# zhouxuguang/GNXRayTracer

Measured on AMD Instinct MI355X. Metric: Mrays/sec + wall-clock to 1024spp, dragon Cornell 1920×1080, higher is better.
Workload: dtype f32; 1 GPU; cfg3: Cornell + synthetic 100000-tri mesh (stand-in for absent dragon.3d), Glass+Metal, PathIntegrator maxDepth 8 rr 1 spatial, Halton(1024), 1920x1080; passes_in_flight=4, sub_passes=56, spp_rendered=1024, gather=n/a, world_size=1, backend=none, devices_visible=1

## Files before the change

gnxraytracer_amd/csrc/api.hip:

```cpp
#include <hip/hip_runtime.h>

#include <chrono>
#include <cstdio>
#include <cstdlib>
#include <memory>
#include <mutex>
#include <string>
#include <thread>
#include <vector>

#include "host_scene.h"
#include "kernels.hip.h"
#include "trace4_kernel.hip.h"
#include "hlbvh_build.hip.h"
#include "refit_kernel.hip.h"
#include "material_kernel.hip.h"
#include "rebuild_kernel.hip.h"
#include "env_build_kernel.hip.h"
#include "media_kernel.hip.h"
#include "texture_build_kernel.hip.h"
#include "li_kernel.hip.h"
#include "views_kernel.hip.h"
#include "shade_query_kernel.hip.h"
#include "aov_kernel.hip.h"
#include "kernel_instances.h"

using namespace gnxr;

#define X(M, L, S, T) extern template GX_WHITTED_SIGNATURE(M, L, S, T)
GX_WHITTED_INSTANCES(X)
#undef X
#define X(M, L, ST, T) extern template GX_VOL_SIGNATURE(M, L, ST, T)
GX_VOL_INSTANCES(X)
#undef X
#define X(M, L) extern template GX_SHADE_KIND_SIGNATURE(M, L)
GX_SHADE_KIND_INSTANCES(X)
#undef X
extern template GX_BSDF_QUERY_SIGNATURE(LM_ALL)
extern template GX_LIGHT_SAMPLE_QUERY_SIGNATURE(LT_ALL)
extern template GX_LIGHT_LE_QUERY_SIGNATURE(LT_ALL)
extern template GX_TRACE_CLOSEST_CODE_SIGNATURE(32)
extern template GX_TRACE_CLOSEST_CODE_SIGNATURE(64)
#define X(M) extern template GX_AOV_RESOLVE_SIGNATURE(M)
GX_AOV_INSTANCES(X)
#undef X

#include "api_common.hip.h"
#include "api_scene.hip.h"
#include "api_hlbvh.hip.h"
#include "api_probes.hip.h"
#include "api_device_call.hip.h"
#include "api_render.hip.h"

extern "C" {

int gnxr_init(int device_id) {
    int n = 0;
    hipError_t e = hipGetDeviceCount(&n);
    if (e != hipSuccess || n <= 0) { set_error("no HIP device available; libgnxr has no CPU fallback"); return GNXR_ERR_NO_DEVICE; }
// ... 394 lines not shown
```

gnxraytracer_amd/csrc/api_common.hip.h:

```cpp
#pragma once

namespace { int hip_status(hipError_t e); }
#define HIP_TRY(expr)                                                                                   \
    do {                                                                                                \
        hipError_t e_ = (expr);                                                                         \
        if (e_ != hipSuccess) {                                                                         \
            set_error("%s failed: %s (%s:%d)", #expr, hipGetErrorString(e_), __FILE__, __LINE__);       \
            return hip_status(e_);                                                                      \
        }                                                                                               \
    } while (0)

namespace {

int hip_status(hipError_t e) {
    if (e == hipErrorOutOfMemory) return GNXR_ERR_OOM;
    if (e == hipErrorNoDevice || e == hipErrorInvalidDevice || e == hipErrorInsufficientDriver || e == hipErrorNotInitialized) return GNXR_ERR_NO_DEVICE;
    return GNXR_ERR_RUNTIME;
}

int g_device = -1;
std::vector<int> g_devices;
std::vector<char> g_peer_ok;
int g_num_cus = 256;
int g_profiling = 0;
// ... 24 lines not shown
struct Knobs {
    static int env_int(const char *name, int unset) { const char *e = getenv(name); return e ? atoi(e) : unset; }
    static bool env_set(const char *name) { return getenv(name) != nullptr; }
#define GX_ONCE(type, expr) do { static const type v = (expr); return v; } while (0)
    static int trace_blocks_per_cu() { const int v = env_int("GNXR_TRACE_BLOCKS_PER_CU", 0); return v >= 1 && v <= 8 ? v : 0; }
    static int grid_blocks_per_cu() { const int v = env_int("GNXR_GRID_BLOCKS_PER_CU", 0); return v >= 1 && v <= 4096 ? v : 0; }
    static int trace_lds_levels() { GX_ONCE(int, env_set("GNXR_TRACE_LDS_LEVELS") ? std::max(2, env_int("GNXR_TRACE_LDS_LEVELS", 0)) : 64); }
    static int trace_chunk() { GX_ONCE(int, env_set("GNXR_TRACE_CHUNK") ? std::max(64, env_int("GNXR_TRACE_CHUNK", 0) / 64 * 64) : kTraceChunk); }
    static bool leaf_box_table() { GX_ONCE(bool, env_set("GNXR_LEAF_BOX_TABLE")); }
    static int regions() { GX_ONCE(int, env_int("GNXR_REGIONS", 0)); }
    static bool pipeline() { GX_ONCE(bool, env_int("GNXR_PIPELINE", 1) != 0); }
    static int pipe_cut() { GX_ONCE(int, env_int("GNXR_PIPE_CUT", -1)); }
    static int loop_lag() { GX_ONCE(int, env_int("GNXR_LOOP_LAG", -1)); }
    static int shade_blocks_per_cu() { GX_ONCE(int, env_set("GNXR_SHADE_BLOCKS_PER_CU") ? std::max(1, env_int("GNXR_SHADE_BLOCKS_PER_CU", 0)) : 32); }
    static int shade_lds_dims() { GX_ONCE(int, env_set("GNXR_SHADE_LDS_DIMS") ? std::max(0, std::min(128, env_int("GNXR_SHADE_LDS_DIMS", 0))) : 64); }
    static bool shade_lds_tables() { GX_ONCE(bool, env_int("GNXR_SHADE_LDS_TABLES", 1) != 0); }
    static int shade_streams() { GX_ONCE(int, env_int("GNXR_SHADE_STREAMS", -1)); }
    static bool vol_pack() { GX_ONCE(bool, env_int("GNXR_VOL_PACK", 1) != 0); }
#undef GX_ONCE
    static int volmedia_step_cap() { return env_set("GNXR_VOLMEDIA_STEP_CAP") ? std::max(0, env_int("GNXR_VOLMEDIA_STEP_CAP", 0)) : 64; }
    static bool no_escape_queue() { return env_set("GNXR_NO_ESCAPE_QUEUE"); }
    static bool no_material_queues() { return env_set("GNXR_NO_MATERIAL_QUEUES"); }
    static bool no_narrow_shade() { return env_set("GNXR_NO_NARROW_SHADE"); }
    static bool host_light_grid() { return env_set("GNXR_HOST_LIGHT_GRID"); }
    static bool binary_bvh() { return env_set("GNXR_BINARY_BVH"); }
};

int ensure_device() {
    if (g_device >= 0) { HIP_TRY(hipSetDevice(g_device)); return GNXR_OK; }
    int n = 0;
    hipError_t e = hipGetDeviceCount(&n);
    if (e != hipSuccess || n <= 0) {
        set_error("no HIP device available (%s); libgnxr has no CPU fallback", e != hipSuccess ? hipGetErrorString(e) : "0 devices");
        return GNXR_ERR_NO_DEVICE;
    }
    int dev = 0;
    HIP_TRY(hipGetDevice(&dev));
    hipDeviceProp_t prop;
    HIP_TRY(hipGetDeviceProperties(&prop, dev));
    g_num_cus = prop.multiProcessorCount > 0 ? prop.multiProcessorCount : 256;
    g_device = dev;
    if (const int v = Knobs::trace_blocks_per_cu()) g_trace_blocks_per_cu = v;
    if (const int v = Knobs::grid_blocks_per_cu()) g_grid_bpc = v;
    return GNXR_OK;
}

// ... 32 lines not shown
```

gnxraytracer_amd/csrc/api_render.hip.h:

```cpp
#pragma once

struct TraceLaunch {
    int entries;
    int lds_entries;
    bool spill_needed;
    size_t lds;
    int n_top;
    int blocks;
};
static TraceLaunch trace_launch(const gnxr_scene *s, bool wide, bool spheres, long long total) {
    TraceLaunch t;
    t.entries = wide ? s->cs.stack4_need + 1 : s->cs.bvh_max_depth + 2;
    const int per_cu = g_trace_blocks_per_cu;
    const size_t fixed_b = wide ? (size_t)(kRayRecDwords + (spheres ? 1 : 0)) * kRqStride * sizeof(int) + (size_t)kTopCache * 128 + kOrderTableBytes : 0;
    t.lds_entries = std::min(std::min(t.entries, Knobs::trace_lds_levels()), std::max(2, (int)(((160 * 1024) / per_cu - 1024 - fixed_b) / (kBlock * sizeof(int)))));
    t.spill_needed = t.entries > t.lds_entries;
    t.lds = (size_t)t.lds_entries * kBlock * sizeof(int) + fixed_b;
    t.n_top = (int)std::min<size_t>(kTopCache, s->cs.root4 >= 0 ? s->cs.nodes4.size() : 0);
    t.blocks = (int)std::min<long long>((long long)g_num_cus * per_cu, (total + kBlock - 1) / kBlock);
    return t;
}

static int count_local_rows(const gnxr_render_params *p) {
    int rows = 0;
// ... 257 lines not shown
        record_ptrs(vol_alt_rec, ps.rec);
        ps.state = vol_alt_state.p; ps.orig = vol_alt_orig.p;
    }
    return ps;
}

struct RenderRun {
    gnxr_scene *s;
    RenderState &st;
    hipStream_t stream;
    const RenderPlan &pl;
    const RaySource *src;
    const ViewSource *views;
    DScene sc;
    DRender r;
    PathArrays pa;
    VolArrays va;
    WhittedArrays wa;
    DMediaTables mt;
    Counters *dctr;
    KernelTimer timer;
    const bool timing = (g_profiling & 1) != 0, count_wide = (g_profiling & 4) != 0, counting = (g_profiling & 2) != 0 && !count_wide;
    bool spheres;
    bool list_media = false;
    int n_lights, n_scene_media;
    unsigned long long rays_closest = 0, rays_any = 0, rays_mis = 0, media_segments = 0;
    unsigned long long new_paths = 0;
    unsigned int launches = 0, passes = 0, loop_iterations = 0;

    RenderRun(gnxr_scene *scene, hipStream_t stream_, const RenderPlan &plan, const RaySource *src_, const ViewSource *views_, const DScene &sc_, const DRender &r_)
        : s(scene), st(scene->st), stream(stream_), pl(plan), src(src_), views(views_), sc(sc_), r(r_), pa(st.path_arrays()), va(st.vol_arrays()),
          wa(st.whitted_arrays(plan, (int)scene->cs.desc_lights.size())), mt(scene->media_tables()), dctr(scene->counters.p), spheres(scene->cs.n_spheres > 0),
          n_lights((int)scene->cs.desc_lights.size()), n_scene_media((int)scene->cs.media.size()) {}

    void launch_trace(TraceWork w, int n_sh, int n_mis, bool count_rays = true);
    void compact(int mode, const int *qin, int nin, const unsigned char *keys, int nout, int nscatter, unsigned int *totals, int *o0, int *o1, int *o2, int *o3 = nullptr, int split = 0,
                 const unsigned *n_dev = nullptr, unsigned kind_queue = 0x01010101u);
    int shade_stage(const int *q_in, int n, int *q_out, const unsigned *n_dev);
    void raygen(const PathArrays &at, long long u0, int kk, unsigned char *medium_keys);
    void resolve(const PathArrays &at, long long u0, int kk);
    void bind_set(const VolPackSet &ps);
};

void RenderRun::launch_trace(TraceWork w, int n_sh, int n_mis, bool count_rays) {
    long long total = (long long)w.n_closest + w.n_nee;
    if (total <= 0) return;
// ... 34 lines not shown
        (void)hipMemsetAsync(st.tile_desc.p, 0, st.tile_desc.n * sizeof(unsigned long long), stream);
        st.compact_seq = 0;
    }
    const unsigned seq = ++st.compact_seq;
    const CompactScratch cs{st.tile_desc.p, tiles, st.compact_ticket.p + (seq & 1u), st.compact_ticket.p + ((seq + 1u) & 1u), seq};
    const bool hitclass = mode == COMPACT_HITCLASS;
    const int *hit = hitclass ? (const int *)st.hit.p : nullptr;
    const unsigned char *cls = hitclass ? (const unsigned char *)s->tri_class.p : nullptr;
#define GX_COMPACT(M, N, NS) hipLaunchKernelGGL((k_compact<M, N, NS>), dim3(g), dim3(kCompactBlock), 0, stream, qin, nin, keys, cs, totals, o0, o1, o2, o3, hit, cls, kind_queue, split, n_dev, dctr)
    if (mode == COMPACT_FLAGS) {
        if (nout == 5) { if (nscatter == 3) GX_COMPACT(COMPACT_FLAGS, 5, 3); else GX_COMPACT(COMPACT_FLAGS, 5, 2); }
        else { if (nscatter == 3) GX_COMPACT(COMPACT_FLAGS, 4, 3); else GX_COMPACT(COMPACT_FLAGS, 4, 2); }
    } else if (hitclass) { if (nout == 4) GX_COMPACT(COMPACT_HITCLASS, 4, 4); else GX_COMPACT(COMPACT_HITCLASS, 3, 3); }
    else if (nout == 4) GX_COMPACT(COMPACT_CLASS, 4, 4);
    else GX_COMPACT(COMPACT_CLASS, 3, 3);
#undef GX_COMPACT
    launches += 1;
}
static int compact_stalled(const Counters &c) {
    if (!c.compact_stall) return GNXR_OK;
    set_error("queue compaction: a tile waited for its predecessors beyond the poll limit (k_compact); the render was abandoned");
    return GNXR_ERR_RUNTIME;
}

int RenderRun::shade_stage(const int *q_in, int n, int *q_out, const unsigned *n_dev) {
    if (timing) timer.begin(2, stream);
    const int *qk = pl.queue_kernel;
    const int n_classes = qk[3] != SHADE_Q_NONE ? 4 : 3;
    compact(COMPACT_HITCLASS, q_in, n, st.pclass.p, n_classes, n_classes, &dctr->q_class[0], st.queue_c0.p, st.queue_c1.p, st.queue_c2.p, st.queue_c3.p, 0, n_dev, pl.kind_queue);
    int *qc[4] = {st.queue_c0.p, st.queue_c1.p, st.queue_c2.p, st.queue_c3.p};
    dim3 g(grid_for(n, Knobs::shade_blocks_per_cu())), b(kBlock);
    const int sdims = std::min<int>(Knobs::shade_lds_dims(), (int)s->cs.prime_sums.size() - 1);
    const int snperm = sdims > 0 ? s->cs.prime_sums[sdims] : 0;
    const bool shade_lds_tabs = Knobs::shade_lds_tables();
    const int lmats = (shade_lds_tabs && s->cs.materials.size() <= 12) ? (int)s->cs.materials.size() : 0;
    const int llights = (shade_lds_tabs && n_lights > 0 && n_lights <= 16) ? n_lights : 0;
    const size_t slds = (sdims > 0 ? ((((size_t)snperm * 2 + 15) & ~(size_t)15) + (size_t)sdims * 32) : 0) + (size_t)lmats * sizeof(DMaterial) + (size_t)llights * sizeof(DLight);
    const int shade_streams = Knobs::shade_streams();
    int n_class_kernels = 0;
    for (int q = 0; q < 4; ++q) n_class_kernels += qk[q] != SHADE_Q_NONE ? 1 : 0;
    const bool fork = (shade_streams < 0 ? n_class_kernels >= 3 : (shade_streams != 0 && n_class_kernels >= 2)) && s->aux_stream[0] && s->aux_stream[1];
    hipStream_t cst[4] = {stream, stream, stream, stream};
    if (fork) {
        HIP_TRY(hipEventRecord(s->ev_fork, stream));
        HIP_TRY(hipStreamWaitEvent(s->aux_stream[0], s->ev_fork, 0));
        HIP_TRY(hipStreamWaitEvent(s->aux_stream[1], s->ev_fork, 0));
        cst[1] = s->aux_stream[0]; cst[2] = s->aux_stream[1]; cst[3] = s->aux_stream[1];
    }
    const bool area_only = pl.area_only, area_env_only = pl.area_env_only;
#define GX_SHADE_K(K, C) hipLaunchKernelGGL(K, g, b, slds, cst[C], sc, r, pa, (const int *)qc[C], (const unsigned int *)&dctr->q_class[C], sdims, snperm, lmats, llights)
#define GX_SHADE(LMV, LTV, C) do { if (spheres) GX_SHADE_K((k_shade<LMV, LTV, true>), C); else GX_SHADE_K((k_shade<LMV, LTV, false>), C); } while (0)
#define GX_SHADE_TEX(LTV) do { if (spheres) GX_SHADE_K((k_shade<LM_ALL, LTV, true, true>), 3); else GX_SHADE_K((k_shade<LM_ALL, LTV, false, true>), 3); } while (0)
    const int light_set = area_only ? 0 : ((area_env_only && !spheres && !(pl.class_mask & 8)) ? 1 : 2);
#define GX_SHADE_LM(LMV, C) do { \
        if (light_set == 0) GX_SHADE(LMV, LT_AREA, C); \
        else if (light_set == 1) GX_SHADE_K((k_shade<LMV, LT_AREA | LT_ENV, false>), C); \
        else GX_SHADE(LMV, LT_ALL, C); } while (0)
#define GX_SHADE_NARROW(LMV, C) do { \
        if (light_set == 0) GX_SHADE_K((k_shade<LMV, LT_AREA, false>), C); \
        else if (light_set == 1) GX_SHADE_K((k_shade<LMV, LT_AREA | LT_ENV, false>), C); \
        else GX_SHADE_K((k_shade<LMV, LT_ALL, false>), C); } while (0)
    for (int q = 0; q < 4; ++q) {
        switch (qk[q]) {
        case SHADE_Q_DIFFUSE: GX_SHADE_LM(LM_DIFFUSE, q); break;
        case SHADE_Q_GLOSSY: GX_SHADE_LM(LM_GLOSSY, q); break;
        case SHADE_Q_CONDUCTOR: GX_SHADE_NARROW(LM_CONDUCTOR, q); break;
        case SHADE_Q_ROUGH_DIELECTRIC: GX_SHADE_NARROW(LM_ROUGH_DIELECTRIC, q); break;
        case SHADE_Q_ALL: GX_SHADE_LM(LM_ALL, q); break;
        case SHADE_Q_TEX: if (light_set == 0) GX_SHADE_TEX(LT_AREA); else GX_SHADE_TEX(LT_ALL); break;
        case SHADE_Q_ESCAPE:
            if (area_env_only) hipLaunchKernelGGL((k_shade_escape<LT_AREA | LT_ENV>), g, b, 0, cst[q], sc, pa, (const int *)qc[q], (const unsigned int *)&dctr->q_class[q]);
            else hipLaunchKernelGGL((k_shade_escape<LT_ALL>), g, b, 0, cst[q], sc, pa, (const int *)qc[q], (const unsigned int *)&dctr->q_class[q]);
            break;
        default: continue;
        }
        ++launches;
    }
#undef GX_SHADE_NARROW
#undef GX_SHADE_LM
#undef GX_SHADE_TEX
#undef GX_SHADE
#undef GX_SHADE_K
    if (fork) {
        HIP_TRY(hipEventRecord(s->ev_join[0], s->aux_stream[0]));
        HIP_TRY(hipEventRecord(s->ev_join[1], s->aux_stream[1]));
        HIP_TRY(hipStreamWaitEvent(stream, s->ev_join[0], 0));
        HIP_TRY(hipStreamWaitEvent(stream, s->ev_join[1], 0));
    }
    compact(COMPACT_FLAGS, q_in, n, st.pflags.p, 4, 2, &dctr->q_next, q_out, st.queue_nee.p, nullptr, nullptr, 0, n_dev);
    if (timing) timer.end(stream);
    return GNXR_OK;
}

void RenderRun::raygen(const PathArrays &at, long long u0, int kk, unsigned char *medium_keys) {
    const int n_new = (int)(pl.unit * kk);
    if (views) hipLaunchKernelGGL(k_raygen_views, dim3(grid_for(n_new)), dim3(kBlock), 0, stream, sc, r, (const DCamera *)st.view_cams.p, at, n_new, (int)u0, medium_keys);
    else if (!src) hipLaunchKernelGGL(k_raygen, dim3(grid_for(n_new)), dim3(kBlock), 0, stream, sc, r, at, n_new, (int)u0);
    else hipLaunchKernelGGL(k_raygen_rays, dim3(grid_for(n_new)), dim3(kBlock), 0, stream, sc, r, at, reinterpret_cast<const float4 *>(src->rays + u0),
                            reinterpret_cast<const int4 *>(src->samples + u0), n_new, n_scene_media, medium_keys, dctr, u0);
}
void RenderRun::resolve(const PathArrays &at, long long u0, int kk) {
    if (!src) hipLaunchKernelGGL(k_resolve, dim3(grid_for(r.npix)), dim3(kBlock), 0, stream, at, st.accum.p, r.npix, kk);
    else hipLaunchKernelGGL(k_store_li, dim3(grid_for(kk)), dim3(kBlock), 0, stream, (const float4 *)at.L, reinterpret_cast<const int4 *>(src->samples + u0), r,
                            n_scene_media, kk, reinterpret_cast<float4 *>(src->L) + u0);
}
// ... 474 lines not shown
```

gnxraytracer_amd/csrc/device_bsdf.h:

```cpp
#pragma once
#include "device_sampler.h"

namespace gnxr {

GX_DEV float cos_theta(V3 w) { return w.z; }
GX_DEV float cos2_theta(V3 w) { return w.z * w.z; }
GX_DEV float abs_cos_theta(V3 w) { return fabsf(w.z); }
GX_DEV float sin2_theta(V3 w) { return fmaxf(0.f, 1.f - cos2_theta(w)); }
GX_DEV float sin_theta(V3 w) { return gx_sqrt(sin2_theta(w)); }
GX_DEV float tan_theta(V3 w) { return sin_theta(w) / cos_theta(w); }
GX_DEV float tan2_theta(V3 w) { return sin2_theta(w) / cos2_theta(w); }
GX_DEV float cos_phi(V3 w) { float s = sin_theta(w); return (s == 0) ? 1 : clampf(w.x / s, -1, 1); }
GX_DEV float sin_phi(V3 w) { float s = sin_theta(w); return (s == 0) ? 0 : clampf(w.y / s, -1, 1); }
GX_DEV float cos2_phi(V3 w) { return cos_phi(w) * cos_phi(w); }
GX_DEV float sin2_phi(V3 w) { return sin_phi(w) * sin_phi(w); }
GX_DEV bool same_hemisphere(V3 w, V3 wp) { return w.z * wp.z > 0; }
GX_DEV V3 reflect(V3 wo, V3 n) { return -wo + 2 * dot(wo, n) * n; }
GX_DEV bool refract(V3 wi, V3 n, float eta, V3 *wt) {
    float cosThetaI = dot(n, wi);
    float sin2ThetaI = fmaxf(0.f, 1 - cosThetaI * cosThetaI);
    float sin2ThetaT = eta * eta * sin2ThetaI;
    if (sin2ThetaT >= 1) return false;
    float cosThetaT = gx_sqrt(1 - sin2ThetaT);
    *wt = eta * -wi + (eta * cosThetaI - cosThetaT) * n;
// ... 340 lines not shown
        float cosTheta = gx_sqrt(fmaxf(0.f, (1 - gx_pow(alpha2, 1 - u0)) / (1 - alpha2)));
        float sinTheta = gx_sqrt(fmaxf(0.f, 1 - cosTheta * cosTheta));
        float phi = 2 * GX_PI * u1;
        float sinPhi, cosPhi;
        gx_sincos(phi, &sinPhi, &cosPhi);
        V3 wh(sinTheta * cosPhi, sinTheta * sinPhi, cosTheta);
        if (!same_hemisphere(wo, wh)) wh = -wh;
        *wi = reflect(wo, wh);
        if (!same_hemisphere(wo, *wi)) return Spec(0.f);
        *pdf = lobe_pdf<LM>(l, wo, *wi);
        return need_f ? lobe_f<LM>(l, wo, *wi) : Spec(0.f);
    }
    break;
    default: break;
    }
    if (lm_micro_only(LM)) return Spec(0.f);
    *wi = cosine_sample_hemisphere(u0, u1);
    if (wo.z < 0) wi->z *= -1;
    *pdf = lobe_pdf<LM>(l, wo, *wi);
    return need_f ? lobe_f<LM>(l, wo, *wi) : Spec(0.f);
}

template <uint32_t LM>
struct Bsdf {
    const DMaterial *mat;
    V3 ns, ng, ss, ts;
    GX_DEV V3 to_local(V3 v) const { return V3(dot(v, ss), dot(v, ts), dot(v, ns)); }
    GX_DEV V3 to_world(V3 v) const {
        return V3(ss.x * v.x + ts.x * v.y + ns.x * v.z, ss.y * v.x + ts.y * v.y + ns.y * v.z, ss.z * v.x + ts.z * v.y + ns.z * v.z);
    }
    GX_DEV static bool matches(int type, int flags) { return (type & flags) == type; }
    GX_DEV int num_components(int flags) const {
        int n = 0;
        for (int i = 0; i < mat->n_lobes; ++i) if (matches(mat->lobes[i].type, flags)) ++n;
        return n;
    }
    static constexpr bool kSingle = (LM == LM_DIFFUSE || LM == LM_CONDUCTOR);
    static constexpr int kSingleType = BSDF_REFLECTION | (LM == LM_CONDUCTOR ? BSDF_GLOSSY : BSDF_DIFFUSE);
    GX_DEV Spec f(V3 woW, V3 wiW, int flags) const {
        V3 wi = to_local(wiW), wo = to_local(woW);
        if (wo.z == 0) return Spec(0.f);
        bool refl = dot(wiW, ng) * dot(woW, ng) > 0;
        if (kSingle) return (mat->n_lobes > 0 && refl && matches(kSingleType, flags)) ? lobe_f<LM>(mat->lobes[0], wo, wi) : Spec(0.f);
        return sum_f(wo, wi, flags, refl);
    }
    GX_DEV Spec sum_f(V3 wo, V3 wi, int flags, bool refl) const {
// ... 4 lines not shown
            while (i < n) {
                const int t = mat->lobes[i].type;
                if (matches(t, flags) && ((refl && (t & BSDF_REFLECTION)) || (!refl && (t & BSDF_TRANSMISSION)))) break;
                ++i;
            }
            if (i >= n) break;
            f = f + lobe_f<LM>(mat->lobes[i], wo, wi);
            ++i;
        }
        return f;
    }
    GX_DEV float pdf(V3 woW, V3 wiW, int flags) const {
        if (mat->n_lobes == 0) return 0.f;
        V3 wo = to_local(woW), wi = to_local(wiW);
        if (wo.z == 0) return 0.f;
        if (kSingle) return matches(kSingleType, flags) ? 0.f + lobe_pdf<LM>(mat->lobes[0], wo, wi) : 0.f;
        float p = 0.f;
        int matching = 0;
        for (int i = 0; i < mat->n_lobes; ++i) {
            const DLobe &l = mat->lobes[i];
            if (matches(l.type, flags)) { ++matching; p += lobe_pdf<LM>(l, wo, wi); }
        }
        return matching > 0 ? p / matching : 0.f;
    }
    GX_DEV Spec sample_f(V3 woW, V3 *wiW, float u0, float u1, float *pdf, int flags, int *sampledType) const {
        if (kSingle) {
            *sampledType = 0;
            if (mat->n_lobes == 0 || !matches(kSingleType, flags)) { *pdf = 0; return Spec(0.f); }
            const DLobe &bx = mat->lobes[0];
            const float ur0 = fminf(u0 * 1 - 0, GX_ONE_MINUS_EPS);
            V3 wi, wo = to_local(woW);
            *pdf = 0;
            if (wo.z == 0) return Spec(0.f);
            *sampledType = kSingleType;
            (void)lobe_sample<LM>(bx, wo, &wi, ur0, u1, pdf, sampledType, false);
            if (*pdf == 0) { *sampledType = 0; return Spec(0.f); }
            *wiW = to_world(wi);
            const bool refl = dot(*wiW, ng) * dot(woW, ng) > 0;
            return refl ? lobe_f<LM>(bx, wo, wi) : Spec(0.f);
        }
        int matching = num_components(flags);
        *sampledType = 0;
        if (matching == 0) { *pdf = 0; return Spec(0.f); }
        int comp = min((int)floorf(u0 * matching), matching - 1);
        int which = -1, count = comp;
        for (int i = 0; i < mat->n_lobes; ++i)
// ... 31 lines not shown
```

gnxraytracer_amd/csrc/inst_shade_kinds.hip:

```cpp
#include "kernel_instances.h"
using namespace gnxr;
#define X(M, L) template GX_SHADE_KIND_SIGNATURE(M, L)
GX_SHADE_KIND_INSTANCES(X)
#undef X
```

gnxraytracer_amd/csrc/kernel_instances.h:

```cpp
#pragma once
#include <hip/hip_runtime.h>

#include "host_scene.h"
#include "kernels.hip.h"
#include "vol_kernel.hip.h"
#include "whitted_kernel.hip.h"

#define GX_WH_SPH(X, M, L, T) X(M, L, false, T) X(M, L, true, T)
#define GX_WH_LT(X, M, T) GX_WH_SPH(X, M, LT_AREA, T) GX_WH_SPH(X, M, LT_ALL, T)
#define GX_WHITTED_INSTANCES_TEX(X, T) GX_WH_LT(X, WM_WHITTED, T) GX_WH_LT(X, WM_DIRECT_ONE, T) GX_WH_LT(X, WM_DIRECT_ALL, T)
#define GX_WHITTED_INSTANCES(X) GX_WHITTED_INSTANCES_TEX(X, false) GX_WHITTED_INSTANCES_TEX(X, true)

#define GX_VS_ST(X, M, L, T) X(M, L, VS_MAIN, T) X(M, L, VS_SHADOW, T) X(M, L, VS_MIS, T)
#define GX_VS_LT(X, M, T) GX_VS_ST(X, M, LT_AREA, T) GX_VS_ST(X, M, LT_ALL, T)
#define GX_VOL_INSTANCES(X) GX_VS_LT(X, LM_DIFFUSE, false) GX_VS_LT(X, LM_GLOSSY, false) GX_VS_LT(X, LM_ALL, false) GX_VS_LT(X, LM_ALL, true)

#define GX_SK_LT(X, M) X(M, LT_AREA) X(M, LT_AREA | LT_ENV) X(M, LT_ALL)
#define GX_SHADE_KIND_INSTANCES(X) GX_SK_LT(X, LM_CONDUCTOR) GX_SK_LT(X, LM_ROUGH_DIELECTRIC)

#define GX_SHADE_KIND_SIGNATURE(M, L) \
    __global__ void gnxr::k_shade<M, L, false, false>(gnxr::DScene, gnxr::DRender, gnxr::PathArrays, const int *, const unsigned int *, int, int, int, int);
#define GX_WHITTED_SIGNATURE(M, L, S, T) \
    __global__ void gnxr::k_whitted_step<M, L, S, T>(gnxr::DScene, gnxr::DRender, gnxr::PathArrays, gnxr::WhittedArrays, const int *, int, unsigned long long *);
#define GX_VOL_SIGNATURE(M, L, ST, T) \
    __global__ void gnxr::k_vol_step<M, L, ST, T>(gnxr::DScene, gnxr::DMediaTables, gnxr::DRender, gnxr::PathArrays, gnxr::VolArrays, const int *, const unsigned int *, int, int);
```

gnxraytracer_amd/csrc/kernels.hip.h:

```cpp
#pragma once
#include "device_bsdf.h"
#include "device_lights.h"
#include "device_texture.h"

namespace gnxr {

constexpr int kBlock = 256;

constexpr int kRS = 2;
constexpr int kRSm = 2 * kRS;
constexpr int kRecGroups = 5;
struct PathArrays {
    float4 *ray_o;
    float4 *ray_d;
    float4 *beta;
    uint2 *meta;
    float4 *L;
    int *hit;
    unsigned char *pflags;
    unsigned char *pclass;
    float4 *sh_o;
    float4 *sh_d;
    float4 *sh_X;
    float4 *nbeta;
// ... 327 lines not shown
#define GX_SHADE_ATTR __attribute__((amdgpu_waves_per_eu(GX_SHADE_MINWAVES)))
#endif
#ifdef GX_SHADE_STATS
static __device__ unsigned long long g_shade_stats[16];
#define GX_STICK(i) do { const unsigned long long t_ = __builtin_amdgcn_s_memtime(); if ((threadIdx.x & 63) == 0) sst_[i] += t_ - stick_; stick_ = t_; } while (0)
#else
#define GX_STICK(i) do {} while (0)
#endif
#ifndef GX_SHADE_W_DIFFUSE
#define GX_SHADE_W_DIFFUSE 3
#endif
#ifndef GX_SHADE_W_GLOSSY
#define GX_SHADE_W_GLOSSY 3
#endif
#ifndef GX_SHADE_W_ALL
#define GX_SHADE_W_ALL GX_SHADE_MINWAVES
#endif
#ifndef GX_SHADE_W_TEX
#define GX_SHADE_W_TEX 3
#endif
template <uint32_t LM> constexpr int shade_min_waves() {
    return LM == LM_DIFFUSE ? GX_SHADE_W_DIFFUSE : ((LM == LM_GLOSSY || LM == LM_CONDUCTOR || LM == LM_ROUGH_DIELECTRIC) ? GX_SHADE_W_GLOSSY : GX_SHADE_W_ALL);
}
template <uint32_t LM, int LT, bool SPH, bool TEX = false>
__global__ void __launch_bounds__(kBlock, (TEX ? GX_SHADE_W_TEX : shade_min_waves<LM>())) k_shade(DScene sc, DRender r, PathArrays pa, const int *__restrict__ queue, const unsigned int *n_dev, int lds_dims, int lds_nperm, int lds_mats, int lds_lights) {
    extern __shared__ int shade_smem[];
    const int n = (int)*n_dev;
    if (blockIdx.x * blockDim.x >= (unsigned)n) return;
    const LdsSampler lsam = lds_sampler_fill(sc.st, lds_dims, lds_nperm, shade_smem, threadIdx.x, kBlock);
    const DMaterial *mats = sc.materials;
    DLightTables ltab = sc.lt;
    {
        int *dst = shade_smem + (lds_sampler_bytes(lds_nperm, lds_dims) >> 2);
        if (!TEX && lds_mats > 0) {
            const int *src = reinterpret_cast<const int *>(sc.materials);
            const int nd = lds_mats * (int)(sizeof(DMaterial) / 4);
            for (int k = threadIdx.x; k < nd; k += kBlock) dst[k] = src[k];
            mats = reinterpret_cast<const DMaterial *>(dst);
            dst += nd;
        }
        if (lds_lights > 0) {
            const int *src = reinterpret_cast<const int *>(sc.lt.lights);
            const int nd = lds_lights * (int)(sizeof(DLight) / 4);
            for (int k = threadIdx.x; k < nd; k += kBlock) dst[k] = src[k];
            ltab.lights = reinterpret_cast<const DLight *>(dst);
        }
    }
    __syncthreads();
#ifdef GX_SHADE_STATS
    unsigned long long sst_[16] = {0};
    unsigned long long stick_ = __builtin_amdgcn_s_memtime();
#endif
    const int stride_ = (int)(gridDim.x * blockDim.x);
    int i = (int)(blockIdx.x * blockDim.x + threadIdx.x);
    int pathCur_ = i < n ? queue[i] : -1;
    int leafCur_ = pathCur_ >= 0 ? pa.hit[pathCur_] : -1;
    int pathNext_ = (long long)i + stride_ < n ? queue[i + stride_] : -1;
    for (; i < n; i += stride_) {
        bool survive = false, wantNee = false, wantShadow = false, wantMis = false;
        int path = -1;
        GX_STICK(9);
        const int leafNext_ = pathNext_ >= 0 ? pa.hit[pathNext_] : -1;
        const int pathNext2_ = (long long)i + 2ll * stride_ < n ? queue[i + 2 * stride_] : -1;
        {
            path = pathCur_;
            uint2 m = pa.meta[(size_t)path * kRSm];
            uint32_t index = m.x;
            int dim = (int)(m.y & 0xffffu), bounces = (int)((m.y >> 16) & 0xffu);
            bool specularBounce = (m.y >> 31) != 0;
            float4 o4 = pa.ray_o[(size_t)path * kRS], d4 = pa.ray_d[(size_t)path * kRS], b4 = pa.beta[(size_t)path * kRS];
            V3 ro(o4.x, o4.y, o4.z), rd(d4.x, d4.y, d4.z);
            Spec beta(b4.x, b4.y, b4.z);
            float etaScale = b4.w;
            int leaf = leafCur_;
            bool found = leaf != -1;
            V3 p0, p1, p2;
            int triMat = -1, triLight = -1;
            TriHit h;
            SurfacePoint sp;
            sp.valid = false;
            found = shade_hit_rebuild<SPH, TEX>(sc, mats, leaf, ro, rd, o4.w, &p0, &p1, &p2, &h, &triMat, &triLight, &sp, nullptr, nullptr);
            GX_STICK(0);
            if ((bounces == 0 || specularBounce) && (found ? triLight >= 0 : ltab.n_infinite > 0)) {
// ... 12 lines not shown
                } else {
                    DMaterial tm;
                    RayDiff none;
                    none.has = false;
                    const DMaterial *mat = shade_material<TEX>(sc, mats + triMat, leaf, p0, p1, p2, h, sp, none, &tm);
                    Bsdf<LM> bsdf;
                    bsdf.mat = mat; bsdf.ns = sp.ns; bsdf.ng = sp.n; bsdf.ss = sp.ss; bsdf.ts = sp.ts;
                    SampleStream ss(sc.st, index, dim, lsam);
                    V3 woN = normalize(-rd);
                    if (mat->n_nonspecular > 0 && ltab.n_lights > 0) {
                        float lightPdfSel;
                        int lightNum = light_select(ltab, sp.p, ss.get1d(), &lightPdfSel);
                        GX_STICK(2);
                        if (lightPdfSel != 0) {
                            float ul0, ul1, us0, us1;
                            ss.get2d(&ul0, &ul1);
                            ss.get2d(&us0, &us1);
                            GX_STICK(3);
                            const int bsdfFlags = BSDF_ALL & ~BSDF_SPECULAR;
                            int nflags = 0;
                            V3 so, sd, mo, wi2;
                            Spec X(0.f), Y(0.f);
                            int expect = -1;
                            LightSample ls = light_sample<LT>(ltab, lightNum, sp.p, ul0, ul1);
                            GX_STICK(4);
                            float scatteringPdf = 0;
                            if (ls.pdf > 0 && !ls.Li.is_black()) {
                                Spec f = bsdf.f(woN, ls.wi, bsdfFlags) * absdot(ls.wi, sp.ns);
                                scatteringPdf = bsdf.pdf(woN, ls.wi, bsdfFlags);
                                if (!f.is_black()) {
                                    spawn_ray_to(sp.p, sp.pError, sp.n, ls.p1, ls.p1Error, ls.n1, &so, &sd);
                                    float weight = light_is_delta<LT>(ltab.lights[lightNum]) ? 1.f : power_heuristic(ls.pdf, scatteringPdf);
                                    X = f * ls.Li * weight / ls.pdf;
                                    nflags |= 1;
                                }
                            }
                            GX_STICK(5);
                            if (!light_is_delta<LT>(ltab.lights[lightNum])) {
                                int sampledType;
                                Spec f = bsdf.sample_f(woN, &wi2, us0, us1, &scatteringPdf, bsdfFlags, &sampledType);
                                f = f * absdot(wi2, sp.ns);
                                bool sampledSpecular = (sampledType & BSDF_SPECULAR) != 0;
                                GX_STICK(6);
                                if (!f.is_black() && scatteringPdf > 0) {
                                    float weight = 1;
                                    bool skip = false;
                                    if (!sampledSpecular) {
                                        float lightPdf = light_pdf<LT>(ltab, lightNum, sp.p, sp.pError, sp.n, wi2);
                                        if (lightPdf == 0) skip = true;
                                        else weight = power_heuristic(scatteringPdf, lightPdf);
                                    }
                                    if (!skip) {
                                        const DLight &lt = ltab.lights[lightNum];
                                        mo = offset_ray_origin(sp.p, sp.pError, sp.n, wi2);
                                        Spec Li2;
                                        if (LT == LT_AREA || lt.type == GNXR_LIGHT_AREA_TRI) {
                                            V3 lp0(lt.p0[0], lt.p0[1], lt.p0[2]), lp1(lt.p1[0], lt.p1[1], lt.p1[2]), lp2(lt.p2[0], lt.p2[1], lt.p2[2]);
                                            V3 ln = normalize(cross(lp0 - lp2, lp1 - lp2));
                                            Li2 = area_L(lt, ln, -wi2);
                                            expect = lt.tri_leaf;
                                        } else {
                                            Li2 = light_Le<LT>(ltab, lightNum, mo, wi2);
                                            expect = -1;
                                        }
                                        if (!Li2.is_black()) Y = f * Li2 * Spec(1.f) * weight / scatteringPdf;
                                        nflags |= 2;
                                    }
                                }
                            }
                            GX_STICK(7);
                            if (nflags) {
                                pa.sh_o[(size_t)path * kRS] = make_float4(so.x, so.y, so.z, 1 - GX_SHADOW_EPS);
                                pa.sh_d[(size_t)path * kRS] = make_float4(sd.x, sd.y, sd.z, __int_as_float(nflags));
                                pa.sh_X[(size_t)path * kRS] = make_float4(X.r, X.g, X.b, lightPdfSel);
                                if (nflags & 2) {
                                    pa.mis_o[(size_t)path * kRS] = make_float4(mo.x, mo.y, mo.z, __int_as_float(expect));
                                    pa.mis_d[(size_t)path * kRS] = make_float4(wi2.x, wi2.y, wi2.z, 0.f);
                                    pa.mis_Y[path] = make_float4(Y.r, Y.g, Y.b, 0.f);
                                }
                                pa.nbeta[(size_t)path * kRS] = make_float4(beta.r, beta.g, beta.b, 0.f);
                                const bool betaFinite = __builtin_isfinite(beta.r) && __builtin_isfinite(beta.g) && __builtin_isfinite(beta.b);
                                pa.nee_vis[path] = ((unsigned)nflags | (betaFinite ? 0u : 0x80u)) << 16;
                                wantNee = true;
                                wantShadow = (nflags & 1) != 0;
                                wantMis = (nflags & 2) != 0;
                            }
                        }
                    }
                    GX_STICK(8);
                    V3 wo = -rd, wi;
                    float pdf, u0, u1;
                    int flags;
                    ss.get2d(&u0, &u1);
                    Spec f = bsdf.sample_f(wo, &wi, u0, u1, &pdf, BSDF_ALL, &flags);
                    if (!(f.is_black() || pdf == 0.f)) {
                        beta = beta * (f * absdot(wi, sp.ns) / pdf);
                        specularBounce = (flags & BSDF_SPECULAR) != 0;
                        if ((flags & BSDF_SPECULAR) && (flags & BSDF_TRANSMISSION)) {
                            float eta = mat->eta;
                            etaScale *= (dot(wo, sp.n) > 0) ? (eta * eta) : 1 / (eta * eta);
                        }
                        V3 o2 = offset_ray_origin(sp.p, sp.pError, sp.n, wi);
                        Spec rrBeta = beta * etaScale;
                        survive = true;
                        if (rrBeta.max_value() < r.rr_threshold && bounces > 3) {
                            float q = fmaxf(.05f, 1 - rrBeta.max_value());
                            if (ss.get1d() < q) survive = false;
                            else beta = beta / (1 - q);
                        }
                        if (survive) {
                            pa.ray_o[(size_t)path * kRS] = make_float4(o2.x, o2.y, o2.z, GX_INF);
                            pa.ray_d[(size_t)path * kRS] = make_float4(wi.x, wi.y, wi.z, d4.w);
                            pa.beta[(size_t)path * kRS] = make_float4(beta.r, beta.g, beta.b, etaScale);
                            pa.store_meta(path, index, (uint32_t)ss.dim | ((uint32_t)(bounces + 1) << 16) | (specularBounce ? 0x80000000u : 0u));
                        }
                    }
                }
            }
            GX_STICK(10);
        }
        pa.pflags[path] = (unsigned char)((survive ? 1 : 0) | (wantNee ? 2 : 0) | (wantShadow ? 4 : 0) | (wantMis ? 8 : 0));
        pathCur_ = pathNext_; leafCur_ = leafNext_; pathNext_ = pathNext2_;
    }
#ifdef GX_SHADE_STATS
    if ((threadIdx.x & 63) == 0) for (int k = 0; k < 16; ++k) if (sst_[k]) atomicAdd(&g_shade_stats[k], sst_[k]);
#endif
}

template <int LT>
__global__ void __launch_bounds__(kBlock) k_shade_escape(DScene sc, PathArrays pa, const int *__restrict__ queue, const unsigned int *n_dev) {
    const int n = (int)*n_dev;
    for (int i = blockIdx.x * blockDim.x + threadIdx.x; i < n; i += gridDim.x * blockDim.x) {
        const int path = queue[i];
        const uint2 m = pa.meta[(size_t)path * kRSm];
        const int bounces = (int)((m.y >> 16) & 0xffu);
        const bool specularBounce = (m.y >> 31) != 0;
        if (bounces == 0 || specularBounce) {
            const float4 o4 = pa.ray_o[(size_t)path * kRS], d4 = pa.ray_d[(size_t)path * kRS], b4 = pa.beta[(size_t)path * kRS], L4 = pa.L[path];
            const V3 ro(o4.x, o4.y, o4.z), rd(d4.x, d4.y, d4.z);
            const Spec beta(b4.x, b4.y, b4.z);
            Spec L(L4.x, L4.y, L4.z);
            for (int k = 0; k < sc.lt.n_infinite; ++k) L = L + beta * light_Le<LT>(sc.lt, sc.lt.infinite[k], ro, rd);
            pa.L[path] = make_float4(L.r, L.g, L.b, 0.f);
        }
// ... 257 lines not shown
```

Baseline: 5310 Mrays/s.

## Defer MIS BSDF-sampling half into per-wave LDS queue to reduce divergence

For area-light-only scenes, the shade kernel now decides up front which lanes need the BSDF-sampled MIS contribution. Instead of evaluating it inline under divergence, it packs each such lane's shading state into a per-wavefront LDS list and drains the list in full-wave batches later. An alternative mode computes the MIS eligibility before light sampling. This aims to cut SIMD lane divergence in the costly sample_f and light_pdf path. In exchange it uses more LDS, which can lower occupancy, adds redundant direction sampling and wave-level fences, and restructures the loop so it terminates via a ballot.

```diff
diff --git a/gnxraytracer_amd/csrc/api.hip b/gnxraytracer_amd/csrc/api.hip
--- a/gnxraytracer_amd/csrc/api.hip
+++ b/gnxraytracer_amd/csrc/api.hip
@@ -35,6 +35,9 @@
 #undef X
 #define X(M, L) extern template GX_SHADE_KIND_SIGNATURE(M, L)
 GX_SHADE_KIND_INSTANCES(X)
+#undef X
+#define X(M, L, S) extern template GX_SHADE_MIS_SIGNATURE(M, L, S)
+GX_SHADE_MIS_INSTANCES(X)
 #undef X
 extern template GX_BSDF_QUERY_SIGNATURE(LM_ALL)
 extern template GX_LIGHT_SAMPLE_QUERY_SIGNATURE(LT_ALL)
diff --git a/gnxraytracer_amd/csrc/api_common.hip.h b/gnxraytracer_amd/csrc/api_common.hip.h
--- a/gnxraytracer_amd/csrc/api_common.hip.h
+++ b/gnxraytracer_amd/csrc/api_common.hip.h
@@ -70,6 +70,9 @@
     static bool no_escape_queue() { return env_set("GNXR_NO_ESCAPE_QUEUE"); }
     static bool no_material_queues() { return env_set("GNXR_NO_MATERIAL_QUEUES"); }
     static bool no_narrow_shade() { return env_set("GNXR_NO_NARROW_SHADE"); }
+    static bool no_mis_defer() { return env_set("GNXR_NO_MIS_DEFER"); }
+    static int mis_defer_step() { const int v = env_int("GNXR_MIS_DEFER_STEP", 2); return v == 1 ? 1 : 2; }
+    static int mis_defer_drain_at() { return std::max(1, std::min(64, env_int("GNXR_MIS_DEFER_DRAIN_AT", 64))); }
     static bool host_light_grid() { return env_set("GNXR_HOST_LIGHT_GRID"); }
     static bool binary_bvh() { return env_set("GNXR_BINARY_BVH"); }
 };
diff --git a/gnxraytracer_amd/csrc/api_render.hip.h b/gnxraytracer_amd/csrc/api_render.hip.h
--- a/gnxraytracer_amd/csrc/api_render.hip.h
+++ b/gnxraytracer_amd/csrc/api_render.hip.h
@@ -303,6 +303,7 @@
     KernelTimer timer;
     const bool timing = (g_profiling & 1) != 0, count_wide = (g_profiling & 4) != 0, counting = (g_profiling & 2) != 0 && !count_wide;
     bool spheres;
+    const int mis_mode = Knobs::no_mis_defer() ? 0 : Knobs::mis_defer_step(), mis_drain_at = Knobs::mis_defer_drain_at();
     bool list_media = false;
     int n_lights, n_scene_media;
     unsigned long long rays_closest = 0, rays_any = 0, rays_mis = 0, media_segments = 0;
@@ -383,6 +384,8 @@
     set_error("queue compaction: a tile waited for its predecessors beyond the poll limit (k_compact); the render was abandoned");
     return GNXR_ERR_RUNTIME;
 }
+
+constexpr size_t kShadeLdsBudget = 52 * 1024;
 
 int RenderRun::shade_stage(const int *q_in, int n, int *q_out, const unsigned *n_dev) {
     if (timing) timer.begin(2, stream);
@@ -409,16 +412,26 @@
         cst[1] = s->aux_stream[0]; cst[2] = s->aux_stream[1]; cst[3] = s->aux_stream[1];
     }
     const bool area_only = pl.area_only, area_env_only = pl.area_env_only;
-#define GX_SHADE_K(K, C) hipLaunchKernelGGL(K, g, b, slds, cst[C], sc, r, pa, (const int *)qc[C], (const unsigned int *)&dctr->q_class[C], sdims, snperm, lmats, llights)
+#define GX_SHADE_KA(K, C, LDS, LL) hipLaunchKernelGGL(K, g, b, LDS, cst[C], sc, r, pa, (const int *)qc[C], (const unsigned int *)&dctr->q_class[C], sdims, snperm, lmats, LL)
+#define GX_SHADE_K(K, C) GX_SHADE_KA(K, C, slds, llights)
 #define GX_SHADE(LMV, LTV, C) do { if (spheres) GX_SHADE_K((k_shade<LMV, LTV, true>), C); else GX_SHADE_K((k_shade<LMV, LTV, false>), C); } while (0)
+#define GX_SHADE_AREA_S(LMV, SPHV, C) do { \
+        if (mis_step == 2) GX_SHADE_KA((k_shade<LMV, LT_AREA | SM_DEFER, SPHV>), C, slds_mis, llights_mis); \
+        else if (mis_step == 1) GX_SHADE_K((k_shade<LMV, LT_AREA | SM_DIR_FIRST, SPHV>), C); \
+        else GX_SHADE_K((k_shade<LMV, LT_AREA, SPHV>), C); } while (0)
+#define GX_SHADE_AREA(LMV, C) do { if (spheres) GX_SHADE_AREA_S(LMV, true, C); else GX_SHADE_AREA_S(LMV, false, C); } while (0)
 #define GX_SHADE_TEX(LTV) do { if (spheres) GX_SHADE_K((k_shade<LM_ALL, LTV, true, true>), 3); else GX_SHADE_K((k_shade<LM_ALL, LTV, false, true>), 3); } while (0)
     const int light_set = area_only ? 0 : ((area_env_only && !spheres && !(pl.class_mask & 8)) ? 1 : 2);
+    int mis_step = light_set == 0 ? mis_mode : 0;
+    const size_t slds_mis = slds + (size_t)(kBlock / 64) * ((size_t)kMisEntryWords * kMisCap + 1) * sizeof(int);
+    const int llights_mis = llights | (std::min(mis_drain_at, kMisCap) << 8);
+    if (mis_step == 2 && slds_mis > kShadeLdsBudget) mis_step = 1;
 #define GX_SHADE_LM(LMV, C) do { \
-        if (light_set == 0) GX_SHADE(LMV, LT_AREA, C); \
+        if (light_set == 0) GX_SHADE_AREA(LMV, C); \
         else if (light_set == 1) GX_SHADE_K((k_shade<LMV, LT_AREA | LT_ENV, false>), C); \
         else GX_SHADE(LMV, LT_ALL, C); } while (0)
 #define GX_SHADE_NARROW(LMV, C) do { \
-        if (light_set == 0) GX_SHADE_K((k_shade<LMV, LT_AREA, false>), C); \
+        if (light_set == 0) GX_SHADE_AREA_S(LMV, false, C); \
         else if (light_set == 1) GX_SHADE_K((k_shade<LMV, LT_AREA | LT_ENV, false>), C); \
         else GX_SHADE_K((k_shade<LMV, LT_ALL, false>), C); } while (0)
     for (int q = 0; q < 4; ++q) {
@@ -440,8 +453,11 @@
 #undef GX_SHADE_NARROW
 #undef GX_SHADE_LM
 #undef GX_SHADE_TEX
+#undef GX_SHADE_AREA
+#undef GX_SHADE_AREA_S
 #undef GX_SHADE
 #undef GX_SHADE_K
+#undef GX_SHADE_KA
     if (fork) {
         HIP_TRY(hipEventRecord(s->ev_join[0], s->aux_stream[0]));
         HIP_TRY(hipEventRecord(s->ev_join[1], s->aux_stream[1]));
diff --git a/gnxraytracer_amd/csrc/device_bsdf.h b/gnxraytracer_amd/csrc/device_bsdf.h
--- a/gnxraytracer_amd/csrc/device_bsdf.h
+++ b/gnxraytracer_amd/csrc/device_bsdf.h
@@ -386,6 +386,51 @@
 }
 
 template <uint32_t LM>
+GX_DEV bool lobe_dir(const DLobe &l, V3 wo, V3 *wi, float u0, float u1) {
+    switch (l.kind) {
+    case LOBE_SPEC_REFL: case LOBE_SPEC_TRANS: case LOBE_FRESNEL_SPEC: return false;
+    case LOBE_MICRO_REFL: case LOBE_MICRO_TRANS: if (GX_HAS_LOBE(LOBE_MICRO_REFL) || GX_HAS_LOBE(LOBE_MICRO_TRANS)) {
+        if (wo.z == 0) return false;
+        V3 wh = tr_sample_wh(l.alphax, l.alphay, wo, u0, u1);
+        if (dot(wo, wh) < 0) return false;
+        if (GX_MICRO_IS_REFL(l)) {
+            *wi = reflect(wo, wh);
+            return same_hemisphere(wo, *wi);
+        }
+        const bool up = cos_theta(wo) > 0;
+        float eta = (up ? l.etaA : l.etaB) / (up ? l.etaB : l.etaA);
+        return refract(wo, wh, eta, wi);
+    }
+    break;
+    case LOBE_LAMBERT_TRANS: if (GX_HAS_LOBE(LOBE_LAMBERT_TRANS)) {
+        *wi = cosine_sample_hemisphere(u0, u1);
+        if (wo.z > 0) wi->z *= -1;
+        return true;
+    }
+    break;
+    case LOBE_DISNEY_CLEARCOAT: if (GX_HAS_LOBE(LOBE_DISNEY_CLEARCOAT)) {
+        if (wo.z == 0) return false;
+        float alpha2 = l.gloss * l.gloss;
+        float cosTheta = gx_sqrt(fmaxf(0.f, (1 - gx_pow(alpha2, 1 - u0)) / (1 - alpha2)));
+        float sinTheta = gx_sqrt(fmaxf(0.f, 1 - cosTheta * cosTheta));
+        float phi = 2 * GX_PI * u1;
+        float sinPhi, cosPhi;
+        gx_sincos(phi, &sinPhi, &cosPhi);
+        V3 wh(sinTheta * cosPhi, sinTheta * sinPhi, cosTheta);
+        if (!same_hemisphere(wo, wh)) wh = -wh;
+        *wi = reflect(wo, wh);
+        return same_hemisphere(wo, *wi);
+    }
+    break;
+    default: break;
+    }
+    if (lm_micro_only(LM)) return false;
+    *wi = cosine_sample_hemisphere(u0, u1);
+    if (wo.z < 0) wi->z *= -1;
+    return true;
+}
+
+template <uint32_t LM>
 struct Bsdf {
     const DMaterial *mat;
     V3 ns, ng, ss, ts;
@@ -436,6 +481,25 @@
             if (matches(l.type, flags)) { ++matching; p += lobe_pdf<LM>(l, wo, wi); }
         }
         return matching > 0 ? p / matching : 0.f;
+    }
+    GX_DEV bool sample_dir(V3 woW, V3 *wiW, float u0, float u1, int flags) const {
+        V3 wi, wo = to_local(woW);
+        if (kSingle) {
+            if (mat->n_lobes == 0 || !matches(kSingleType, flags) || wo.z == 0) return false;
+            if (!lobe_dir<LM>(mat->lobes[0], wo, &wi, fminf(u0 * 1 - 0, GX_ONE_MINUS_EPS), u1)) return false;
+        } else {
+            const int matching = num_components(flags);
+            if (matching == 0) return false;
+            int comp = min((int)floorf(u0 * matching), matching - 1);
+            int which = -1, count = comp;
+            for (int i = 0; i < mat->n_lobes; ++i)
+                if (matches(mat->lobes[i].type, flags) && count-- == 0) { which = i; break; }
+            float ur0 = fminf(u0 * matching - comp, GX_ONE_MINUS_EPS);
+            if (wo.z == 0) return false;
+            if (!lobe_dir<LM>(mat->lobes[which], wo, &wi, ur0, u1)) return false;
+        }
+        *wiW = to_world(wi);
+        return true;
     }
     GX_DEV Spec sample_f(V3 woW, V3 *wiW, float u0, float u1, float *pdf, int flags, int *sampledType) const {
         if (kSingle) {
diff --git a/gnxraytracer_amd/csrc/inst_shade_kinds.hip b/gnxraytracer_amd/csrc/inst_shade_kinds.hip
--- a/gnxraytracer_amd/csrc/inst_shade_kinds.hip
+++ b/gnxraytracer_amd/csrc/inst_shade_kinds.hip
@@ -3,3 +3,6 @@
 #define X(M, L) template GX_SHADE_KIND_SIGNATURE(M, L)
 GX_SHADE_KIND_INSTANCES(X)
 #undef X
+#define X(M, L, S) template GX_SHADE_MIS_SIGNATURE(M, L, S)
+GX_SHADE_MIS_INSTANCES(X)
+#undef X
diff --git a/gnxraytracer_amd/csrc/kernel_instances.h b/gnxraytracer_amd/csrc/kernel_instances.h
--- a/gnxraytracer_amd/csrc/kernel_instances.h
+++ b/gnxraytracer_amd/csrc/kernel_instances.h
@@ -18,6 +18,12 @@
 #define GX_SK_LT(X, M) X(M, LT_AREA) X(M, LT_AREA | LT_ENV) X(M, LT_ALL)
 #define GX_SHADE_KIND_INSTANCES(X) GX_SK_LT(X, LM_CONDUCTOR) GX_SK_LT(X, LM_ROUGH_DIELECTRIC)
 
+#define GX_SM_LM(X, L) X(LM_DIFFUSE, L, false) X(LM_DIFFUSE, L, true) X(LM_GLOSSY, L, false) X(LM_GLOSSY, L, true) X(LM_ALL, L, false) X(LM_ALL, L, true) \
+    X(LM_CONDUCTOR, L, false) X(LM_ROUGH_DIELECTRIC, L, false)
+#define GX_SHADE_MIS_INSTANCES(X) GX_SM_LM(X, LT_AREA | SM_DIR_FIRST) GX_SM_LM(X, LT_AREA | SM_DEFER)
+
+#define GX_SHADE_MIS_SIGNATURE(M, L, S) \
+    __global__ void gnxr::k_shade<M, L, S, false>(gnxr::DScene, gnxr::DRender, gnxr::PathArrays, const int *, const unsigned int *, int, int, int, int);
 #define GX_SHADE_KIND_SIGNATURE(M, L) \
     __global__ void gnxr::k_shade<M, L, false, false>(gnxr::DScene, gnxr::DRender, gnxr::PathArrays, const int *, const unsigned int *, int, int, int, int);
 #define GX_WHITTED_SIGNATURE(M, L, S, T) \
diff --git a/gnxraytracer_amd/csrc/kernels.hip.h b/gnxraytracer_amd/csrc/kernels.hip.h
--- a/gnxraytracer_amd/csrc/kernels.hip.h
+++ b/gnxraytracer_amd/csrc/kernels.hip.h
@@ -373,8 +373,63 @@
 template <uint32_t LM> constexpr int shade_min_waves() {
     return LM == LM_DIFFUSE ? GX_SHADE_W_DIFFUSE : ((LM == LM_GLOSSY || LM == LM_CONDUCTOR || LM == LM_ROUGH_DIELECTRIC) ? GX_SHADE_W_GLOSSY : GX_SHADE_W_ALL);
 }
-template <uint32_t LM, int LT, bool SPH, bool TEX = false>
+constexpr int kMisEntryWords = 27, kMisCap = 64;
+template <uint32_t LM>
+GX_DEV void mis_drain_entry(const int *e, const DMaterial *mats, const DLightTables &ltab, const PathArrays &pa) {
+    constexpr int cap = kMisCap;
+#define GX_MF(w) __int_as_float(e[(w) * cap])
+    const int path = e[0], lightNum = e[25 * cap], bits = e[26 * cap];
+    Bsdf<LM> bsdf;
+    bsdf.mat = mats + e[1 * cap];
+    const V3 woN(GX_MF(2), GX_MF(3), GX_MF(4));
+    const float us0 = GX_MF(5), us1 = GX_MF(6);
+    bsdf.ns = V3(GX_MF(7), GX_MF(8), GX_MF(9)); bsdf.ng = V3(GX_MF(10), GX_MF(11), GX_MF(12));
+    bsdf.ss = V3(GX_MF(13), GX_MF(14), GX_MF(15)); bsdf.ts = V3(GX_MF(16), GX_MF(17), GX_MF(18));
+    const V3 p(GX_MF(19), GX_MF(20), GX_MF(21)), pError(GX_MF(22), GX_MF(23), GX_MF(24));
+#undef GX_MF
+    const int bsdfFlags = BSDF_ALL & ~BSDF_SPECULAR;
+    float scatteringPdf = 0;
+    V3 wi2;
+    int sampledType;
+    Spec f = bsdf.sample_f(woN, &wi2, us0, us1, &scatteringPdf, bsdfFlags, &sampledType);
+    f = f * absdot(wi2, bsdf.ns);
+    bool sampledSpecular = (sampledType & BSDF_SPECULAR) != 0;
+    if (!f.is_black() && scatteringPdf > 0) {
+        float weight = 1;
+        bool skip = false;
+        if (!sampledSpecular) {
+            float lightPdf = light_pdf<LT_AREA>(ltab, lightNum, p, pError, bsdf.ng, wi2);
+            if (lightPdf == 0) skip = true;
+            else weight = power_heuristic(scatteringPdf, lightPdf);
+        }
+        if (!skip) {
+            const DLight &lt = ltab.lights[lightNum];
+            V3 mo = offset_ray_origin(p, pError, bsdf.ng, wi2);
+            V3 lp0(lt.p0[0], lt.p0[1], lt.p0[2]), lp1(lt.p1[0], lt.p1[1], lt.p1[2]), lp2(lt.p2[0], lt.p2[1], lt.p2[2]);
+            V3 ln = normalize(cross(lp0 - lp2, lp1 - lp2));
+            Spec Li2 = area_L(lt, ln, -wi2);
+            const int expect = lt.tri_leaf;
+            Spec Y(0.f);
+            if (!Li2.is_black()) Y = f * Li2 * Spec(1.f) * weight / scatteringPdf;
+            const int nflags = (bits & 1) | 2;
+            pa.mis_o[(size_t)path * kRS] = make_float4(mo.x, mo.y, mo.z, __int_as_float(expect));
+            pa.mis_d[(size_t)path * kRS] = make_float4(wi2.x, wi2.y, wi2.z, 0.f);
+            pa.mis_Y[path] = make_float4(Y.r, Y.g, Y.b, 0.f);
+            pa.sh_d[(size_t)path * kRS].w = __int_as_float(nflags);
+            pa.nee_vis[path] = ((unsigned)nflags | ((bits & 2) ? 0u : 0x80u)) << 16;
+            pa.pflags[path] = (unsigned char)(((bits >> 2) & 1) | 2 | ((bits & 1) ? 4 : 0) | 8);
+        }
+    }
+}
+
+constexpr int SM_DIR_FIRST = 16, SM_DEFER = 32;
+template <uint32_t LM, int LTM, bool SPH, bool TEX = false>
 __global__ void __launch_bounds__(kBlock, (TEX ? GX_SHADE_W_TEX : shade_min_waves<LM>())) k_shade(DScene sc, DRender r, PathArrays pa, const int *__restrict__ queue, const unsigned int *n_dev, int lds_dims, int lds_nperm, int lds_mats, int lds_lights) {
+    constexpr int LT = LTM & LT_ALL, MD = LTM >> 4;
+    static_assert(MD == 0 || (LT == LT_AREA && !TEX && MD <= 2), "the MIS half is reordered for area lights without image textures only");
+    constexpr int misCap = kMisCap;
+    const int misDrainAt = MD == 2 ? (lds_lights >> 8) & 0xff : 0;
+    if (MD == 2) lds_lights &= 0xff;
     extern __shared__ int shade_smem[];
     const int n = (int)*n_dev;
     if (blockIdx.x * blockDim.x >= (unsigned)n) return;
@@ -407,9 +462,32 @@
     int pathCur_ = i < n ? queue[i] : -1;
     int leafCur_ = pathCur_ >= 0 ? pa.hit[pathCur_] : -1;
     int pathNext_ = (long long)i + stride_ < n ? queue[i + stride_] : -1;
-    for (; i < n; i += stride_) {
+    int *const misList = shade_smem + (MD != 2 ? 0 : (lds_sampler_bytes(lds_nperm, lds_dims) >> 2) + (lds_mats > 0 ? lds_mats * (int)(sizeof(DMaterial) / 4) : 0) +
+                                                     lds_lights * (int)(sizeof(DLight) / 4) + (int)(threadIdx.x >> 6) * (kMisEntryWords * misCap + 1));
+    int *const misFill = misList + kMisEntryWords * misCap;
+    if (MD == 2) {
+        if ((threadIdx.x & 63) == 0) *misFill = 0;
+        __builtin_amdgcn_fence(__ATOMIC_SEQ_CST, "wavefront");
+    }
+    for (; MD == 2 || i < n; i += stride_) {
         bool survive = false, wantNee = false, wantShadow = false, wantMis = false;
         int path = -1;
+        int misSlot = -1, misBits = 0;
+        if (MD == 2) {
+            const bool act_ = i < n;
+            const bool anyAct_ = __ballot(act_) != 0;
+            __builtin_amdgcn_fence(__ATOMIC_SEQ_CST, "wavefront");
+            const int fill_ = *misFill;
+            if (fill_ > 0 && (fill_ >= misDrainAt || !anyAct_)) {
+                if ((int)(threadIdx.x & 63) < fill_) mis_drain_entry<LM>(misList + (threadIdx.x & 63), mats, ltab, pa);
+                __builtin_amdgcn_fence(__ATOMIC_SEQ_CST, "wavefront");
+                if ((threadIdx.x & 63) == 0) *misFill = 0;
+                __builtin_amdgcn_fence(__ATOMIC_SEQ_CST, "wavefront");
+                GX_STICK(12);
+            }
+            if (!anyAct_) break;
+            if (!act_) { i = n - stride_; continue; }
+        }
         GX_STICK(9);
         const int leafNext_ = pathNext_ >= 0 ? pa.hit[pathNext_] : -1;
         const int pathNext2_ = (long long)i + 2ll * stride_ < n ? queue[i + 2 * stride_] : -1;
@@ -468,6 +546,12 @@
                             V3 so, sd, mo, wi2;
                             Spec X(0.f), Y(0.f);
                             int expect = -1;
+                            bool misLaneEarly_ = true;
+                            if (MD == 1) {
+                                V3 wd;
+                                misLaneEarly_ = bsdf.sample_dir(woN, &wd, us0, us1, bsdfFlags) && light_pdf<LT>(ltab, lightNum, sp.p, sp.pError, sp.n, wd) != 0;
+                                GX_STICK(11);
+                            }
                             LightSample ls = light_sample<LT>(ltab, lightNum, sp.p, ul0, ul1);
                             GX_STICK(4);
                             float scatteringPdf = 0;
@@ -482,7 +566,38 @@
                                 }
                             }
                             GX_STICK(5);
-                            if (!light_is_delta<LT>(ltab.lights[lightNum])) {
+                            bool misLane = !light_is_delta<LT>(ltab.lights[lightNum]);
+                            if (MD == 1) misLane = misLaneEarly_;
+                            if (MD == 2 && misLane) {
+                                V3 wd;
+                                misLane = bsdf.sample_dir(woN, &wd, us0, us1, bsdfFlags) && light_pdf<LT>(ltab, lightNum, sp.p, sp.pError, sp.n, wd) != 0;
+                                GX_STICK(11);
+                            }
+                            if (MD == 2) {
+                                const unsigned long long hm_ = __ballot(misLane);
+                                if (hm_ != 0) {
+                                    const int lane_ = (int)(threadIdx.x & 63), base_ = *misFill;
+                                    const int slot_ = base_ + __popcll(hm_ & ((1ull << lane_) - 1ull));
+                                    if (misLane && slot_ < misCap) {
+                                        int *e_ = misList + slot_;
+#define GX_ME(w, v) e_[(w) * misCap] = (v)
+#define GX_MEF(w, v) e_[(w) * misCap] = __float_as_int(v)
+                                        GX_ME(0, path); GX_ME(1, triMat); GX_MEF(2, woN.x); GX_MEF(3, woN.y); GX_MEF(4, woN.z); GX_MEF(5, us0); GX_MEF(6, us1);
+                                        GX_MEF(7, sp.ns.x); GX_MEF(8, sp.ns.y); GX_MEF(9, sp.ns.z); GX_MEF(10, sp.n.x); GX_MEF(11, sp.n.y); GX_MEF(12, sp.n.z);
+                                        GX_MEF(13, sp.ss.x); GX_MEF(14, sp.ss.y); GX_MEF(15, sp.ss.z); GX_MEF(16, sp.ts.x); GX_MEF(17, sp.ts.y); GX_MEF(18, sp.ts.z);
+                                        GX_MEF(19, sp.p.x); GX_MEF(20, sp.p.y); GX_MEF(21, sp.p.z); GX_MEF(22, sp.pError.x); GX_MEF(23, sp.pError.y); GX_MEF(24, sp.pError.z);
+                                        GX_ME(25, lightNum);
+#undef GX_MEF
+#undef GX_ME
+                                        misSlot = slot_;
+                                        misLane = false;
+                                    }
+                                    __builtin_amdgcn_fence(__ATOMIC_SEQ_CST, "wavefront");
+                                    if (lane_ == __ffsll((long long)hm_) - 1) *misFill = min(base_ + __popcll(hm_), misCap);
+                                    __builtin_amdgcn_fence(__ATOMIC_SEQ_CST, "wavefront");
+                                }
+                            }
+                            if (misLane) {
                                 int sampledType;
                                 Spec f = bsdf.sample_f(woN, &wi2, us0, us1, &scatteringPdf, bsdfFlags, &sampledType);
                                 f = f * absdot(wi2, sp.ns);
@@ -515,7 +630,7 @@
                                 }
                             }
                             GX_STICK(7);
-                            if (nflags) {
+                            if (nflags || (MD == 2 && misSlot >= 0)) {
                                 pa.sh_o[(size_t)path * kRS] = make_float4(so.x, so.y, so.z, 1 - GX_SHADOW_EPS);
                                 pa.sh_d[(size_t)path * kRS] = make_float4(sd.x, sd.y, sd.z, __int_as_float(nflags));
                                 pa.sh_X[(size_t)path * kRS] = make_float4(X.r, X.g, X.b, lightPdfSel);
@@ -527,7 +642,8 @@
                                 pa.nbeta[(size_t)path * kRS] = make_float4(beta.r, beta.g, beta.b, 0.f);
                                 const bool betaFinite = __builtin_isfinite(beta.r) && __builtin_isfinite(beta.g) && __builtin_isfinite(beta.b);
                                 pa.nee_vis[path] = ((unsigned)nflags | (betaFinite ? 0u : 0x80u)) << 16;
-                                wantNee = true;
+                                wantNee = MD == 2 ? nflags != 0 : true;
+                                if (MD == 2) misBits = (nflags & 1) | (betaFinite ? 2 : 0);
                                 wantShadow = (nflags & 1) != 0;
                                 wantMis = (nflags & 2) != 0;
                             }
@@ -566,6 +682,7 @@
             GX_STICK(10);
         }
         pa.pflags[path] = (unsigned char)((survive ? 1 : 0) | (wantNee ? 2 : 0) | (wantShadow ? 4 : 0) | (wantMis ? 8 : 0));
+        if (MD == 2 && misSlot >= 0) misList[26 * misCap + misSlot] = misBits | (survive ? 4 : 0);
         pathCur_ = pathNext_; leafCur_ = leafNext_; pathNext_ = pathNext2_;
     }
 #ifdef GX_SHADE_STATS
```

Result: faster. 5372 Mrays/s, median of 6 (+1.2%).
